# george-gca/sr-pytorch-lightning

Measured on AMD Instinct MI355X. Metric: SR training throughput, LR patches/s (48x48 LR x4, fwd+bwd+Adam), higher is better.
Workload: dtype bf16; 1 GPU; edsr_baseline x4, 48x48 LR patches, batch 256/GPU, train step (L1 + Adam); global_batch=256, parallelism=dp1, hip_graph=full

## Files before the change

### include/srk.h

```cpp
#ifndef SRK_H
#define SRK_H

#include <stdint.h>

#ifdef __cplusplus
extern "C" {
#endif

typedef void* srk_stream_t;

enum { SRK_BF16 = 0, SRK_F16 = 1, SRK_F32 = 2 };

enum {
  SRK_E_BADARG = -1,
  SRK_E_NODEV = -2
};

enum {
  SRK_OUT_NHWC = 0,
  SRK_OUT_NHWC_PS = 1,
  SRK_OUT_PLANAR = 2
};

typedef struct {
// ... 120 lines not shown
  int dtype;
} srk_pw_wgrad_args;
int srk_pw_wgrad_ranges(long long P, int Chid);
int srk_pw_wgrad(const srk_pw_wgrad_args* a, srk_stream_t stream);

typedef struct {
  const void* x; int x_pitch, x_coff; int x_ps;
  const void* dy; int dy_pitch, dy_coff; int dy_ps;
  int N, H, W;
  int Cin, Cout;
  int KH, KW;
  float* dwp;
  float* dbp;
  int nslabs;
  int dtype;
  int cout_real;
} srk_wgrad_args;
int srk_conv2d_wgrad(const srk_wgrad_args* a, srk_stream_t stream);
int srk_wgrad_slabs(const srk_wgrad_args* a);
int srk_wgrad_slab_cout(const srk_wgrad_args* a);

typedef struct {
  const float* dwp; const float* dbp;
  int nslabs;
  float* dw; float* db;
  int Cout, Cin, KH, KW;
  int CinP, CoutP;
  int ps_r;
  float scale;
  int accumulate;
} srk_wgrad_fin_args;
int srk_wgrad_finalize(const srk_wgrad_fin_args* a, srk_stream_t stream);

int srk_wgrad_group_ok(const srk_wgrad_args* a);
int srk_wgrad_group_job_bytes(void);
int srk_wgrad_group_plan(srk_wgrad_args* jobs, int n, float* scratch, void* table_host, int* block_job_host,
                         int* nblocks, long long* scratch_floats);
int srk_conv2d_wgrad_group(const void* table_dev, const int* block_job_dev, int nblocks, int dtype, srk_stream_t stream);
int srk_wgrad_finalize_group(const srk_wgrad_fin_args* table_dev, int n, int blocks_per_job, srk_stream_t stream);
int srk_upload_small(void* dst_dev, const void* src_host, long long nbytes, srk_stream_t stream);
int srk_upload_prepare(void);
int srk_upload_eager(void* dst_dev, const void* src_host, long long nbytes);
int srk_upload_fence(void);

typedef struct {
  const float* x;
  const float* sub;
  void* dst; int dst_pitch, dst_coff;
  int N, Cin, H, W, KH, KW;
  int Kstore;
  int dtype;
} srk_unfold_args;
int srk_unfold_nchw(const srk_unfold_args* a, srk_stream_t stream);

typedef struct {
  const float* src; void* dst; int dst_pitch, dst_coff;
  int N, C, H, W;
  int Cstore; int ps_r; float scale; int dtype;
} srk_to_nhwc_args;
int srk_nchw_to_nhwc(const srk_to_nhwc_args* a, srk_stream_t stream);

typedef struct {
  const void* src; int src_pitch, src_coff; float* dst;
  int N, C, H, W; int dtype;
} srk_to_nchw_args;
int srk_nhwc_to_nchw(const srk_to_nchw_args* a, srk_stream_t stream);

int srk_ca_splits(int N, int HW);
typedef struct {
  const void* t; int t_pitch, t_coff;
  const void* u; int u_pitch, u_coff;
  float* sums;
  int N, HW, C; int dtype;
} srk_ca_pool_args;
int srk_ca_pool(const srk_ca_pool_args* a, srk_stream_t stream);

typedef struct {
  const void* t; int t_pitch, t_coff;
  const void* res; int res_pitch, res_coff;
  const float* sums;
  const float* w1; const float* b1; const float* w2; const float* b2;
  float* s_out; float* z_out;
  void* out; int out_pitch, out_coff;
  int N, HW, C, Cr; int dtype;
  int sums_rows;
} srk_ca_apply_args;
int srk_ca_apply(const srk_ca_apply_args* a, srk_stream_t stream);

typedef struct {
  const void* g; int g_pitch, g_coff;
  const float* gsum;
  const float* sums; const float* s; const float* z;
  const float* w1; const float* w2;
  float* dw1; float* db1; float* dw2; float* db2;
  void* gt; int gt_pitch, gt_coff;
  int N, HW, C, Cr; int dtype;
  int sums_rows, gsum_rows;
} srk_ca_bwd_args;
int srk_ca_bwd_apply(const srk_ca_bwd_args* a, srk_stream_t stream);
typedef struct { const float* src; float* dst; int n; int k; } srk_rowsum_job;
int srk_rowsum_group(const srk_rowsum_job* table_dev, int njobs, int max_k, srk_stream_t stream);

typedef struct {
  const uint8_t* lr; const uint8_t* hr;
  int lr_h, lr_w, hr_h, hr_w;
  int top, left;
// ... 387 lines not shown
```

### sr-pytorch-lightning_amd/csrc/pack.hip

```cpp
#include <stdarg.h>
#include <string.h>
#include <mutex>
#include "srk_common.h"

static thread_local char g_err[512] = "";

void srk_set_error(const char* fmt, ...) {
  va_list ap;
  va_start(ap, fmt);
  vsnprintf(g_err, sizeof(g_err), fmt, ap);
  va_end(ap);
}

extern "C" const char* srk_last_error(void) { return g_err; }
thread_local const char* srk_kernel_name = "";
extern "C" const char* srk_last_kernel(void) { return srk_kernel_name; }
extern "C" int srk_version(void) { return 100; }
extern "C" int srk_device_cus(void) {
  int dev = 0;
  if (hipGetDevice(&dev) != hipSuccess) return 0;
  hipDeviceProp_t p;
  if (hipGetDeviceProperties(&p, dev) != hipSuccess) return 0;
  return p.multiProcessorCount;
}
// ... 371 lines not shown
  const int ncob = (a.CoutP + 63) / 64, ncib = (a.CinP + 1) / 2;
  for (int t = blockIdx.x; t < ncob * ncib; t += gridDim.x) {
    const int cob = t % ncob, cib = t / ncob;
    wgrad_finalize3x3_tile(a, tile, cib * 2, cob * 64);
  }
  if (a.db && a.dbp && blockIdx.x == 0) {
    const int ns = a.nslabs > 1 ? a.nslabs : 1;
    for (int cop = threadIdx.x; cop < a.Cout; cop += blockDim.x) {
      float u = 0.f;
#pragma unroll 8
      for (int sl = 0; sl < ns; ++sl) u += a.dbp[(size_t)sl * a.CoutP + cop];
      int co = cop;
      if (a.ps_r > 1) {
        const int r2p = a.ps_r * a.ps_r, Cc = a.Cout / r2p;
        const int ij = cop / Cc, c = cop - ij * Cc;
        co = c * r2p + ij;
      }
      const float v = a.scale * u;
      if (a.accumulate) a.db[co] += v; else a.db[co] = v;
    }
  }
}

template <int DT> __global__ void to_nhwc_kernel(const srk_to_nhwc_args a) {
  typedef DTraits<DT> Tr;
  typename Tr::elem* dst = reinterpret_cast<typename Tr::elem*>(a.dst);
  const int r = a.ps_r > 1 ? a.ps_r : 1, r2 = r * r;
  const int groups = a.Cstore / 4;
  const long long total = (long long)a.N * a.H * a.W * groups;
  const int Cs = a.C / r2;
  for (long long idx = (long long)blockIdx.x * blockDim.x + threadIdx.x; idx < total; idx += (long long)gridDim.x * blockDim.x) {
    const int g = (int)(idx % groups);
    long long p = idx / groups;
    const int x = (int)(p % a.W);
    p /= a.W;
    const int y = (int)(p % a.H);
    const int n = (int)(p / a.H);
    float v[4];
#pragma unroll
    for (int e = 0; e < 4; ++e) {
      const int c = g * 4 + e;
      float s = 0.f;
      if (c < a.C) {
        const int cs = c / r2, ij = c - cs * r2;
        const int si = ij / r, sj = ij - si * r;
        s = a.scale * a.src[((size_t)(n * Cs + cs) * (a.H * r) + y * r + si) * (a.W * r) + x * r + sj];
      }
      v[e] = s;
    }
    store4<DT>(dst + ((size_t)(n * a.H + y) * a.W + x) * a.dst_pitch + a.dst_coff + g * 4, v);
  }
}

template <int DT> __global__ void to_nhwc16_kernel(const srk_to_nhwc_args a) {
  typedef DTraits<DT> Tr;
  typename Tr::elem* dst = reinterpret_cast<typename Tr::elem*>(a.dst);
  const int r = a.ps_r > 1 ? a.ps_r : 1, r2 = r * r;
  const int Cs = a.C / r2;
  const long long total = (long long)a.N * a.H * a.W;
  for (long long p = (long long)blockIdx.x * blockDim.x + threadIdx.x; p < total; p += (long long)gridDim.x * blockDim.x) {
    const int x = (int)(p % a.W);
    long long q = p / a.W;
    const int y = (int)(q % a.H);
    const int n = (int)(q / a.H);
    float v[16];
#pragma unroll
    for (int c = 0; c < 16; ++c) {
      float s = 0.f;
      if (c < a.C) {
        const int cs = c / r2, ij = c - cs * r2;
        const int si = ij / r, sj = ij - si * r;
        s = a.scale * a.src[((size_t)(n * Cs + cs) * (a.H * r) + y * r + si) * (a.W * r) + x * r + sj];
      }
      v[c] = s;
    }
    typename Tr::elem* o = dst + (size_t)p * a.dst_pitch + a.dst_coff;
    if (Tr::IS16 && (a.dst_pitch & 7) == 0 && (a.dst_coff & 7) == 0) {
#pragma unroll
      for (int g = 0; g < 2; ++g) {
        i32x4 raw;
        raw.x = (int)pack2<DT>(v[8 * g + 0], v[8 * g + 1]); raw.y = (int)pack2<DT>(v[8 * g + 2], v[8 * g + 3]);
        raw.z = (int)pack2<DT>(v[8 * g + 4], v[8 * g + 5]); raw.w = (int)pack2<DT>(v[8 * g + 6], v[8 * g + 7]);
        *reinterpret_cast<i32x4*>(o + 8 * g) = raw;
      }
    } else {
#pragma unroll
      for (int g = 0; g < 4; ++g) store4<DT>(o + 4 * g, v + 4 * g);
    }
  }
}

template <int DT> __global__ void to_nchw_kernel(const srk_to_nchw_args a) {
  typedef DTraits<DT> Tr;
  const typename Tr::elem* src = reinterpret_cast<const typename Tr::elem*>(a.src);
  const long long total = (long long)a.N * a.C * a.H * a.W;
  for (long long idx = (long long)blockIdx.x * blockDim.x + threadIdx.x; idx < total; idx += (long long)gridDim.x * blockDim.x) {
    const int x = (int)(idx % a.W);
    long long t = idx / a.W;
    const int y = (int)(t % a.H);
    t /= a.H;
    const int c = (int)(t % a.C);
    const int n = (int)(t / a.C);
    a.dst[idx] = Tr::to_f32(src[((size_t)(n * a.H + y) * a.W + x) * a.src_pitch + a.src_coff + c]);
  }
}

template <int DT> __global__ void unfold_kernel(const srk_unfold_args a) {
  typedef DTraits<DT> Tr;
  typename Tr::elem* dst = reinterpret_cast<typename Tr::elem*>(a.dst);
  const int groups = a.Kstore / 4, taps = a.KH * a.KW, K = a.Cin * taps;
  const int ph = a.KH / 2, pw = a.KW / 2;
  const long long total = (long long)a.N * a.H * a.W * groups;
  for (long long idx = (long long)blockIdx.x * blockDim.x + threadIdx.x; idx < total; idx += (long long)gridDim.x * blockDim.x) {
    const int g = (int)(idx % groups);
    long long p = idx / groups;
    const int x = (int)(p % a.W);
    p /= a.W;
    const int y = (int)(p % a.H);
    const int n = (int)(p / a.H);
    float v[4];
#pragma unroll
    for (int e = 0; e < 4; ++e) {
      const int k = g * 4 + e;
      float s = 0.f;
      if (k < K) {
        const int ci = k / taps, t = k - ci * taps;
        const int kh = t / a.KW, kw = t - kh * a.KW;
        const int yy = y + kh - ph, xx = x + kw - pw;
        if (yy >= 0 && yy < a.H && xx >= 0 && xx < a.W) {
          s = a.x[((size_t)(n * a.Cin + ci) * a.H + yy) * a.W + xx];
          if (a.sub) s -= a.sub[ci];
        }
      }
      v[e] = s;
    }
    store4<DT>(dst + ((size_t)(n * a.H + y) * a.W + x) * a.dst_pitch + a.dst_coff + g * 4, v);
  }
}

inline int grid_for(long long total, int block) {
// ... 91 lines not shown
constexpr int kMaxDev = 64;
std::mutex g_upload_mu;
hipStream_t g_upload_stream[kMaxDev] = {};
int upload_stream_of_current_device(hipStream_t* out, bool create) {
  int dev = -1;
  hipError_t e = hipGetDevice(&dev);
  if (e != hipSuccess || dev < 0 || dev >= kMaxDev) { srk_set_error("srk_upload: hipGetDevice: %s (device %d)", hipGetErrorString(e), dev); return e != hipSuccess ? (int)e : SRK_E_BADARG; }
  std::lock_guard<std::mutex> lock(g_upload_mu);
  if (!g_upload_stream[dev] && create) {
    e = hipStreamCreateWithFlags(&g_upload_stream[dev], hipStreamNonBlocking);
    if (e != hipSuccess) { g_upload_stream[dev] = nullptr; srk_set_error("srk_upload_prepare: %s", hipGetErrorString(e)); return (int)e; }
  }
  *out = g_upload_stream[dev];
  return 0;
}
}
extern "C" int srk_upload_prepare(void) {
  hipStream_t st = nullptr;
  return upload_stream_of_current_device(&st, true);
}
extern "C" int srk_upload_eager(void* dst_dev, const void* src_host, long long nbytes) {
  hipStream_t st = nullptr;
  const int rc = upload_stream_of_current_device(&st, false);
  if (rc != 0) return rc;
  SRK_CHECK_ARG(st != nullptr, "srk_upload_eager: call srk_upload_prepare() on this device first (outside the capture)");
  return srk_upload_small(dst_dev, src_host, nbytes, reinterpret_cast<srk_stream_t>(st));
}
extern "C" int srk_upload_fence(void) {
  hipStream_t st = nullptr;
  const int rc = upload_stream_of_current_device(&st, false);
  if (rc != 0) return rc;
  if (!st) return 0;
  const hipError_t e = hipStreamSynchronize(st);
  if (e != hipSuccess) { srk_set_error("srk_upload_fence: %s", hipGetErrorString(e)); return (int)e; }
  return 0;
}

extern "C" int srk_wgrad_finalize_group(const srk_wgrad_fin_args* table_dev, int n, int blocks_per_job, srk_stream_t stream) {
  SRK_CHECK_ARG(table_dev && n > 0 && n <= 65535, "srk_wgrad_finalize_group: bad table (%d entries)", n);
  const int bx = blocks_per_job < 1 ? 1 : (blocks_per_job > 2048 ? 2048 : blocks_per_job);
  hipLaunchKernelGGL(wgrad_finalize_group_kernel, dim3(bx, n), dim3(256), 0, reinterpret_cast<hipStream_t>(stream), table_dev);
  SRK_LAUNCH_CHECK();
  return 0;
}

extern "C" int srk_nchw_to_nhwc(const srk_to_nhwc_args* a, srk_stream_t stream) {
  SRK_CHECK_ARG(a && a->src && a->dst, "srk_nchw_to_nhwc: null pointer");
  const int r = a->ps_r > 1 ? a->ps_r : 1;
  SRK_CHECK_ARG(a->Cstore % 4 == 0 && a->Cstore >= a->C && a->C % (r * r) == 0 && a->dst_pitch % 4 == 0 && a->dst_coff % 4 == 0,
                "srk_nchw_to_nhwc: C=%d Cstore=%d r=%d", a->C, a->Cstore, r);
  hipStream_t st = reinterpret_cast<hipStream_t>(stream);
  if (a->Cstore == 16) {
    const long long px = (long long)a->N * a->H * a->W;
    const int g16 = (int)((px + 255) / 256 > 8192 ? 8192 : (px + 255) / 256);
    switch (a->dtype) {
      case SRK_BF16: hipLaunchKernelGGL(to_nhwc16_kernel<SRK_BF16>, dim3(g16), dim3(256), 0, st, *a); break;
      case SRK_F16: hipLaunchKernelGGL(to_nhwc16_kernel<SRK_F16>, dim3(g16), dim3(256), 0, st, *a); break;
      case SRK_F32: hipLaunchKernelGGL(to_nhwc16_kernel<SRK_F32>, dim3(g16), dim3(256), 0, st, *a); break;
      default: SRK_CHECK_ARG(false, "srk_nchw_to_nhwc: dtype %d", a->dtype);
    }
    SRK_LAUNCH_CHECK();
    return 0;
  }
  const long long total = (long long)a->N * a->H * a->W * (a->Cstore / 4);
  const int grid = grid_for(total, 256);
  switch (a->dtype) {
    case SRK_BF16: hipLaunchKernelGGL(to_nhwc_kernel<SRK_BF16>, dim3(grid), dim3(256), 0, st, *a); break;
    case SRK_F16: hipLaunchKernelGGL(to_nhwc_kernel<SRK_F16>, dim3(grid), dim3(256), 0, st, *a); break;
    case SRK_F32: hipLaunchKernelGGL(to_nhwc_kernel<SRK_F32>, dim3(grid), dim3(256), 0, st, *a); break;
    default: SRK_CHECK_ARG(false, "srk_nchw_to_nhwc: dtype %d", a->dtype);
  }
  SRK_LAUNCH_CHECK();
  return 0;
}

extern "C" int srk_nhwc_to_nchw(const srk_to_nchw_args* a, srk_stream_t stream) {
  SRK_CHECK_ARG(a && a->src && a->dst, "srk_nhwc_to_nchw: null pointer");
  const long long total = (long long)a->N * a->C * a->H * a->W;
  hipStream_t st = reinterpret_cast<hipStream_t>(stream);
  const int grid = grid_for(total, 256);
  switch (a->dtype) {
    case SRK_BF16: hipLaunchKernelGGL(to_nchw_kernel<SRK_BF16>, dim3(grid), dim3(256), 0, st, *a); break;
    case SRK_F16: hipLaunchKernelGGL(to_nchw_kernel<SRK_F16>, dim3(grid), dim3(256), 0, st, *a); break;
    case SRK_F32: hipLaunchKernelGGL(to_nchw_kernel<SRK_F32>, dim3(grid), dim3(256), 0, st, *a); break;
    default: SRK_CHECK_ARG(false, "srk_nhwc_to_nchw: dtype %d", a->dtype);
  }
  SRK_LAUNCH_CHECK();
  return 0;
}

template <int DT> __global__ __launch_bounds__(256) void unfold3x3c3_kernel(const srk_unfold_args a) {
  typedef DTraits<DT> Tr;
  static_assert(Tr::IS16, "16-bit storage");
  typename Tr::elem* dst = reinterpret_cast<typename Tr::elem*>(a.dst);
  const long long total = (long long)a.N * a.H * a.W;
  const float sub[3] = {a.sub ? a.sub[0] : 0.f, a.sub ? a.sub[1] : 0.f, a.sub ? a.sub[2] : 0.f};
  for (long long p = (long long)blockIdx.x * 256 + threadIdx.x; p < total; p += (long long)gridDim.x * 256) {
    const int x = (int)(p % a.W);
    const long long q = p / a.W;
    const int y = (int)(q % a.H);
    const int n = (int)(q / a.H);
    float v[32];
#pragma unroll
    for (int ci = 0; ci < 3; ++ci) {
      const float* const plane = a.x + (size_t)(n * 3 + ci) * a.H * a.W;
#pragma unroll
// ... 52 lines not shown
```

### sr-pytorch-lightning_amd/ops.py

```python
import weakref

import torch

from . import _lib as L
from .packing import *
from .packing import _DT, _TLS, _f32c, _group_for, _knob, _need_gpu, _ptr, _roundup, _stream, _tok


def _pitch(t):
    n, h, w, c = t.shape
    p = t.stride(2) if w > 1 else (t.stride(1) if h > 1 else (t.stride(0) if n > 1 else c))
    if w > 1 and h > 1:
        assert t.stride(1) == w * p, "NHWC view must be dense in W"
    if h > 1 and n > 1:
        assert t.stride(0) == h * w * p, "NHWC view must be dense in H"
    assert c == 1 or t.stride(3) == 1, "channels must be innermost"
    return p


_ADDR_LIMIT = 0x7fff0000


def _batch_chunks(n, *tensors):
    worst = 0
# ... 221 lines not shown
            assert c % 16 == 0, "fused PixelShuffle store needs C % 16 == 0"
            out = torch.empty((n, h * ps_r, wd * ps_r, c), dtype=x.dtype, device=x.device)
            conv_raw(x, pk, N=n, H=h, W=wd, Cin=cinp, Cout=cout, out=out, out_mode=L.OUT_NHWC_PS, ps_r=ps_r,
                     scale=scale, res=res)
        else:
            out = torch.empty((n, h, wd, pad16(cout)), dtype=x.dtype, device=x.device)
            conv_raw(x, pk, N=n, H=h, W=wd, Cin=cinp, Cout=out.shape[3], out=out, scale=scale, res=res)
        ctx.save_for_backward(x, w)
        ctx.cfg = (scale, ps_r, b is not None, res is not None)
        ctx.wb = (w, b)
        ctx.pg = _tok()
        ctx.gacc = x.__dict__.get("_srk_gacc")
        return out

    @staticmethod
    def backward(ctx, g):
        x, w = ctx.saved_tensors
        scale, ps_r, has_b, has_res = ctx.cfg
        g = g.contiguous()
        n, h, wd, cinp = x.shape
        cout, cin, k, _ = w.shape
        coutp = pad16(cout)
        gx = gw = gb = None
        if ctx.needs_input_grad[0]:
            pkd = pack_conv(w, None, x.dtype, dgrad=True, ps_r=ps_r, token=ctx.pg)
            if ctx.gacc is not None and ps_r <= 1:
                gx, add = ctx.gacc[0].grad_dest(ctx.gacc[1])
                conv_raw(g, pkd, N=n, H=h, W=wd, Cin=coutp, Cout=cinp, out=gx, scale=scale, use_bias=False, res=gx if add else None)
            else:
                gx = torch.empty_like(x)
                parked = None
                if ctx.link is not None and ctx.link.g is not None:
                    parked, ctx.link.g = ctx.link.g, None
                conv_raw(g, pkd, N=n, H=h, W=wd, Cin=coutp, Cout=cinp, out=gx, scale=scale, x_ps=ps_r, use_bias=False, res=parked)
        if ctx.needs_input_grad[1] or ctx.needs_input_grad[2]:
            gw, gb = wgrad(x, g, wparam=ctx.wb[0], bparam=ctx.wb[1], N=n, H=h, W=wd, Cin=cinp, Cout=coutp, k=k,
                           w_shape=tuple(w.shape), ps_r=ps_r, scale=scale, dy_ps=ps_r, want_bias=has_b)
            gw = gw if ctx.needs_input_grad[1] else None
        return gx, gw, gb, (g if has_res else None), None, None, None


def conv(x, w, b, *, res=None, scale=1.0, ps_r=0, link=None):
    return ConvFn.apply(x, w, b, res, float(scale), int(ps_r), link)


class HeadConvFn(torch.autograd.Function):

    @staticmethod
    def forward(ctx, x, w, b, sub, dtype):
        _need_gpu(x)
        cout, cin, k, _ = w.shape
        n, c, h, wd = x.shape
        assert c == cin
        xu = unfold_raw(x, sub, k, dtype)
        pk = _pack_head(w, b, dtype)
        out = torch.empty((n, h, wd, pad16(cout)), dtype=dtype, device=x.device)
        conv_raw(xu, pk, N=n, H=h, W=wd, Cin=xu.shape[3], Cout=out.shape[3], out=out)
        ctx.save_for_backward(xu, w)
        ctx.has_b = b is not None
        return out

    @staticmethod
    def backward(ctx, g):
        xu, w = ctx.saved_tensors
        g = g.contiguous()
        n, h, wd, kp = xu.shape
        gw = gb = None
        if ctx.needs_input_grad[1] or ctx.needs_input_grad[2]:
            gw, gb = wgrad_raw(xu, g, N=n, H=h, W=wd, Cin=kp, Cout=g.shape[3], k=1, w_shape=tuple(w.shape),
                               want_bias=ctx.has_b)
            gw = gw if ctx.needs_input_grad[1] else None
        return None, gw, gb, None, None


def _pack_head(w, b, dtype):
    return pack_conv(w, b, dtype, as_1x1=True)


def head_conv(x, w, b, sub, dtype):
    return HeadConvFn.apply(x, w, b, sub, dtype)


class TailConvFn(torch.autograd.Function):

    @staticmethod
    def forward(ctx, x, w, b, res, post_add, ps_r):
        _need_gpu(x)
        n, h, wd, cinp = x.shape
        cout, cin, k, _ = w.shape
        r = ps_r if ps_r > 1 else 1
        pk = pack_conv(w, b, x.dtype)
        out = torch.empty((n, cout // (r * r), h * r, wd * r), dtype=torch.float32, device=x.device)
        resc = None if res is None else _f32c(res)
        conv_raw(x, pk, N=n, H=h, W=wd, Cin=cinp, Cout=cout, out=out, out_mode=L.OUT_PLANAR, ps_r=ps_r,
                 res=resc, post_add=post_add)
        ctx.save_for_backward(x, w)
        ctx.cfg = (ps_r, b is not None, res is not None)
        ctx.wb = (w, b)
        ctx.pg = _tok()
        return out

    @staticmethod
    def backward(ctx, g):
        x, w = ctx.saved_tensors
        ps_r, has_b, has_res = ctx.cfg
        n, h, wd, cinp = x.shape
        cout, cin, k, _ = w.shape
        dy = to_nhwc(g, x.dtype, ps_r=ps_r)
        gx = gw = gb = None
        if ctx.needs_input_grad[0]:
            pkd = pack_conv(w, None, x.dtype, dgrad=True, token=ctx.pg)
            gx = torch.empty_like(x)
            conv_raw(dy, pkd, N=n, H=h, W=wd, Cin=dy.shape[3], Cout=cinp, out=gx, use_bias=False)
        if ctx.needs_input_grad[1] or ctx.needs_input_grad[2]:
            gw, gb = wgrad(x, dy, wparam=ctx.wb[0], bparam=ctx.wb[1], N=n, H=h, W=wd, Cin=cinp, Cout=dy.shape[3], k=k,
                           w_shape=tuple(w.shape), want_bias=has_b)
            gw = gw if ctx.needs_input_grad[1] else None
        return gx, gw, gb, (g if has_res else None), None, None


def tail_conv(x, w, b, *, res=None, post_add=None, ps_r=0):
    return TailConvFn.apply(x, w, b, res, post_add, int(ps_r))


class SkipConvFn(torch.autograd.Function):

    @staticmethod
    def forward(ctx, x, w, b, sub, ps_r, dtype):
        _need_gpu(x)
# ... 930 lines not shown
```

### sr-pytorch-lightning_amd/csrc/conv_wgrad.hip

```cpp
#include <stdlib.h>
#include <mutex>
#include "srk_common.h"

namespace {

template <int DT, int KS> struct WgCfg {
  typedef DTraits<DT> Tr;
  static constexpr int CH = Tr::CH;
  static constexpr int ESZ = 16 / CH;
  static constexpr int CBLK = 128 / ESZ;
  static constexpr int RB = CBLK / 32;
  static constexpr int PAIRS = RB * RB;
  static constexpr int KGROUPS = 4 / PAIRS;
  static constexpr int NT = 256;
  static constexpr int NTAPS = KS * KS;
  static constexpr int PAD = KS / 2;
  static constexpr int TIN = 16 + KS - 1;
  static constexpr int PITCH = (TIN + 1) & ~1;
  static constexpr int XS_BYTES = TIN * PITCH * 128;
  static constexpr int DYS_BYTES = 256 * 128;
  static constexpr int LDS_BYTES = XS_BYTES + DYS_BYTES;
  static constexpr int XPIECES = TIN * TIN * 8;
  static constexpr int DYPIECES = 256 * 8;
};
// ... 308 lines not shown
      for (int t = 0; t < 9; ++t) {
        const int kh = t / KS, kw = t - kh * KS;
        acc[t] = Tr::mma(xf[(y + kh) & 3][kw], bf, acc[t]);
        if (t == 1 && 2 * y < NPK && more) dma_x_piece(nxt, 2 * y);
        if (t == 4 && 2 * y + 1 < NPK && more) dma_x_piece(nxt, 2 * y + 1);
        if (t == 7 && y < NDK && more) dma_d_piece(nxt, y);
      }
      bf = bfn;
      __builtin_amdgcn_sched_barrier(0);
    }
  }

  {
    const int co = cob * 64 + cbk * 32 + (lane & 31);
    const int hq = lane >> 5;
    const size_t slab_elems = (size_t)9 * a.Cin * a.Cout;
    const __amdgpu_buffer_rsrc_t srs =
        __builtin_amdgcn_make_buffer_rsrc(a.dwp + (size_t)slot * slab_elems, 0, (unsigned)(slab_elems * 4), 0x00020000);
    const int ci0 = cib * 64 + rb * 32 + 4 * hq;
#pragma unroll
    for (int t = 0; t < 9; ++t) {
#pragma unroll
      for (int e = 0; e < 16; ++e) {
        const int ci = ci0 + (e & 3) + 8 * (e >> 2);
        const unsigned voff = (ci < a.Cin && co < a.Cout) ? (unsigned)(((t * a.Cin + ci) * a.Cout + co) * 4) : 0x80000000u;
        __builtin_amdgcn_raw_buffer_store_b32(__float_as_uint(acc[t][e]), srs, voff, 0, 0);
      }
    }
  }
  if (do_bias) {
    float* const bred = reinterpret_cast<float*>(smem);
    __syncthreads();
#pragma unroll
    for (int e = 0; e < 8; ++e) bred[tid * 8 + e] = bsum8[e];
    __syncthreads();
    if (tid < 64) {
      const int ch = tid >> 3, e = tid & 7;
      float t = 0.f;
      for (int p0 = 0; p0 < 32; ++p0) t += bred[((p0 << 3) + (ch ^ swz(p0 & 15))) * 8 + e];
      const int c = cob * 64 + tid;
      if (c < a.Cout) a.dbp[(size_t)slot * a.Cout + c] = t;
    }
  }
}


constexpr int WS_TH = 8;

SRK_DEV void add_f32_unpacked(float& s, float v) { asm("v_add_f32_e32 %0, %0, %1" : "+v"(s) : "v"(v)); }

#ifndef SRK_WG_STAMPS
#define SRK_WG_STAMPS 0
#endif
#ifndef SRK_WG_HELPER_SLEEP
#define SRK_WG_HELPER_SLEEP 0
#endif
#ifndef SRK_WG_COMPUTE_PRIO
#define SRK_WG_COMPUTE_PRIO 0
#endif
constexpr int WS8_THREADS = 512;

template <int DT, bool BIAS>
SRK_DEV void wgrad_ws_body8(const srk_wgrad_args& a, const int slot, const int cib, const int cob, const int tilesX, const int tilesY,
                           const unsigned x_bytes, const unsigned dy_bytes, const int tq, const int trem, char* const smem, const bool single) {
  typedef WgCfg<DT, 3> C;
  typedef typename C::Tr Tr;
  constexpr int CH = C::CH, KS = 3, GT = 256, ESZ = C::ESZ;
  constexpr int TH = WS_TH, NBUF = 4, AHEAD = NBUF - 1;
  constexpr int XPIECES = (TH + 2) * C::TIN * 8;
  constexpr int NPK = (XPIECES + GT - 1) / GT;
  constexpr int NDK = TH * 16 * 8 / GT;
  constexpr int PPT = NPK + NDK;
  constexpr int XS_PAD = NPK * GT * 16, DYS = TH * 16 * 128;
  constexpr int BUF_BYTES = XS_PAD + DYS;
  static_assert(NBUF * BUF_BYTES <= 160 * 1024, "the ring must fit the LDS");

  const int wave = __builtin_amdgcn_readfirstlane((int)threadIdx.x >> 6);
  const int t0 = slot * tq + min(slot, trem);
  const int nt = tq + (slot < trem ? 1 : 0);
#if SRK_WG_STAMPS
  unsigned long long* const stamp = (single && slot == 0 && cib == 0 && cob == 0 && (threadIdx.x & 255) == 0 && a.dbp)
                                        ? reinterpret_cast<unsigned long long*>(a.dbp + (size_t)a.nslabs * a.Cout) + (wave >> 2) * 64 : nullptr;
#define SRK_GSTAMP(i) do { if (stamp && it < 32) stamp[it * 2 + (i)] = __builtin_amdgcn_s_memtime(); } while (0)
#else
#define SRK_GSTAMP(i) do { } while (0)
#endif

  if (wave >= 4) {
    const int tid = (int)threadIdx.x - GT, hw = wave - 4;
    const int H = a.H, W = a.W;
    const int nch_x = a.Cin / CH, nch_d = a.Cout / CH;
    const i32x4 xrs = make_rsrc4(a.x, x_bytes), drs = make_rsrc4(a.dy, dy_bytes);
    const unsigned lds0 = lds_addr_of(smem);
    int pconst[NPK], pyx[NPK];
#pragma unroll
    for (int k = 0; k < NPK; ++k) {
      const int i = tid + k * GT;
      const int sl = i & 7, p = i >> 3;
      const int iy = p / C::TIN, ix = p - iy * C::TIN;
      const int c = cib * 8 + (sl ^ swz(ix));
      pconst[k] = (((iy - 1) * W + (ix - 1)) * a.x_pitch + a.x_coff + c * CH) * ESZ;
      pyx[k] = (i < XPIECES && c < nch_x) ? (((iy - 1) & 0xffff) | ((ix - 1) << 16)) : (int)0x7fff7fff;
    }
    const int rd = a.dy_ps > 1 ? a.dy_ps : 1;
    const int d_ix = (tid >> 3) & 15, d_iy0 = tid >> 7;
    const int d_c = cob * 8 + ((tid & 7) ^ swz(d_ix));
    const bool d_cok = d_c < nch_d;
    int dconst, dkstride;
    {
      const int Csd = a.Cout / (rd * rd);
      const int k0 = d_c * CH;
      const int ij = k0 / Csd, c0 = k0 - ij * Csd;
      const int si = ij / rd, sj = ij - si * rd;
      dconst = (((d_iy0 * rd + si) * (W * rd) + d_ix * rd + sj) * a.dy_pitch + a.dy_coff + c0) * ESZ;
      dkstride = 2 * rd * (W * rd) * a.dy_pitch * ESZ;
    }
    struct TileAddr { int y0, x0, xbase, dbase; bool colok, live; unsigned Xb; };
    int nx_tX = t0 % tilesX, nx_tY = (t0 / tilesX) % tilesY, nx_n = (t0 / tilesX) / tilesY;
    auto dma_tile = [&](int it_) {
      TileAddr t;
      t.live = it_ < nt;
      t.y0 = nx_tY * TH; t.x0 = nx_tX * 16;
      const int row = nx_n * H + t.y0;
      t.xbase = ((row * W + t.x0) * a.x_pitch) * ESZ;
      t.dbase = ((row * rd * (W * rd) + t.x0 * rd) * a.dy_pitch) * ESZ;
      t.colok = t.live && d_cok && (t.x0 + d_ix < W);
      t.Xb = lds0 + (unsigned)((it_ & (NBUF - 1)) * BUF_BYTES);
      const bool wx = nx_tX + 1 == tilesX;
      nx_tX = wx ? 0 : nx_tX + 1;
      nx_tY += wx ? 1 : 0;
      const bool wy = nx_tY == tilesY;
      nx_tY = wy ? 0 : nx_tY;
      nx_n += wy ? 1 : 0;
#pragma unroll
      for (int k = 0; k < NPK; ++k) {
        const int gy = t.y0 + (int)(short)(pyx[k] & 0xffff), gx = t.x0 + (pyx[k] >> 16);
        const bool ok = t.live && (unsigned)gy < (unsigned)H && (unsigned)gx < (unsigned)W;
        const unsigned voff = ok ? (unsigned)(t.xbase + pconst[k]) : 0x80000000u;
        dma16_hidden(xrs, voff, __builtin_amdgcn_readfirstlane(t.Xb + ((k * GT + hw * 64) << 4)));
        if (SRK_WG_HELPER_SLEEP) __builtin_amdgcn_s_sleep(SRK_WG_HELPER_SLEEP);
      }
#pragma unroll
      for (int k = 0; k < NDK; ++k) {
        const bool ok = t.colok && (t.y0 + d_iy0 + 2 * k < H);
        const unsigned voff = ok ? (unsigned)(t.dbase + dconst + k * dkstride) : 0x80000000u;
        dma16_hidden(drs, voff, __builtin_amdgcn_readfirstlane(t.Xb + XS_PAD + ((k * GT + hw * 64) << 4)));
        if (SRK_WG_HELPER_SLEEP) __builtin_amdgcn_s_sleep(SRK_WG_HELPER_SLEEP);
      }
    };
    float bsum8[8] = {0.f, 0.f, 0.f, 0.f, 0.f, 0.f, 0.f, 0.f};

#pragma unroll
    for (int k = 0; k < AHEAD; ++k) dma_tile(k);
    asm volatile("s_waitcnt vmcnt(%0)" :: "n"((AHEAD - 1) * PPT) : "memory");
    __builtin_amdgcn_s_barrier();
#pragma unroll 1
    for (int it = 0; it < nt; ++it) {
      SRK_GSTAMP(0);
      dma_tile(it + AHEAD);
      if (BIAS) {
        const char* const Ds = smem + (it & (NBUF - 1)) * BUF_BYTES + XS_PAD;
#pragma unroll
        for (int k = 0; k < NDK; ++k) {
          const i32x4 braw = lds_read16(Ds + ((tid + 256 * k) << 4));
#pragma unroll
          for (int i = 0; i < 4; ++i) {
            const uint32_t w = (uint32_t)braw[i];
            add_f32_unpacked(bsum8[2 * i], Tr::to_f32((uint16_t)(w & 0xffff)));
            add_f32_unpacked(bsum8[2 * i + 1], Tr::to_f32((uint16_t)(w >> 16)));
          }
        }
      }
      asm volatile("s_waitcnt lgkmcnt(0)\n\ts_waitcnt vmcnt(%0)" :: "n"((AHEAD - 1) * PPT) : "memory");
      SRK_GSTAMP(1);
      __builtin_amdgcn_s_barrier();
    }
    asm volatile("s_waitcnt vmcnt(0)" ::: "memory");
    if (BIAS) {
      float* const bred = reinterpret_cast<float*>(smem);
      __syncthreads();
#pragma unroll
      for (int e = 0; e < 8; ++e) bred[tid * 8 + e] = bsum8[e];
      __syncthreads();
      if (tid < 64) {
        const int ch = tid >> 3, e = tid & 7;
        float t = 0.f;
        for (int p0 = 0; p0 < 32; ++p0) t += bred[((p0 << 3) + (ch ^ swz(p0 & 15))) * 8 + e];
        const int c = cob * 64 + tid;
        if (c < a.Cout) a.dbp[(size_t)slot * a.Cout + c] = t;
      }
    }
    return;
  }

  const int tid = threadIdx.x, lane = tid & 63;
  const int rb = wave >> 1, cbk = wave & 1;
  f32x16 acc[9];
#pragma unroll
  for (int t = 0; t < 9; ++t)
#pragma unroll
    for (int e = 0; e < 16; ++e) acc[t][e] = 0.f;
  int xoff[KS][2], doff[2];
#pragma unroll
  for (int kw = 0; kw < KS; ++kw) {
    xoff[kw][0] = tr_lane_off(kw, 0, rb, lane);
    xoff[kw][1] = tr_lane_off(kw, 1, rb, lane);
  }
  doff[0] = tr_lane_off(0, 0, cbk, lane);
  doff[1] = tr_lane_off(0, 1, cbk, lane);
  i32x4 pxf[3][KS], pbf;
  auto read_first_frags = [&](const char* Xb) {
    const char* const Db = Xb + XS_PAD;
    pbf = tr_read2(Db + doff[0], Db + doff[1]);
#pragma unroll
    for (int rr = 0; rr < 3; ++rr)
#pragma unroll
      for (int kw = 0; kw < KS; ++kw)
        pxf[rr][kw] = tr_read2(Xb + xoff[kw][0] + rr * (C::PITCH * 128), Xb + xoff[kw][1] + rr * (C::PITCH * 128));
  };

  if (SRK_WG_COMPUTE_PRIO) __builtin_amdgcn_s_setprio(SRK_WG_COMPUTE_PRIO);
  asm volatile("" ::: "memory");
  __builtin_amdgcn_s_barrier();
  asm volatile("" ::: "memory");
  read_first_frags(smem);
#pragma unroll 1
  for (int it = 0; it < nt; ++it) {
    SRK_GSTAMP(0);
    const char* const Xs = smem + (it & (NBUF - 1)) * BUF_BYTES;
    const char* const Ds = Xs + XS_PAD;
    const char* const Xn = smem + ((it + 1) & (NBUF - 1)) * BUF_BYTES;
    i32x4 xf[4][KS];
#pragma unroll
    for (int rr = 0; rr < 3; ++rr)
#pragma unroll
      for (int kw = 0; kw < KS; ++kw) xf[rr][kw] = pxf[rr][kw];
    i32x4 bf = pbf;
#pragma unroll
    for (int y = 0; y < TH; ++y) {
      i32x4 bfn = bf;
      if (y + 1 < TH) {
        const int nr = y + 3;
#pragma unroll
        for (int kw = 0; kw < KS; ++kw)
          xf[nr & 3][kw] = tr_read2(Xs + xoff[kw][0] + nr * (C::PITCH * 128), Xs + xoff[kw][1] + nr * (C::PITCH * 128));
        bfn = tr_read2(Ds + doff[0] + (y + 1) * (16 * 128), Ds + doff[1] + (y + 1) * (16 * 128));
      }
#pragma unroll
      for (int t = 0; t < 9; ++t) {
        const int kh = t / KS, kw = t - kh * KS;
        acc[t] = Tr::mma(xf[(y + kh) & 3][kw], bf, acc[t]);
        if (y == TH - 1 && t == 0) {
          __builtin_amdgcn_sched_barrier(0);
          asm volatile("s_waitcnt lgkmcnt(0)" ::: "memory");
          SRK_GSTAMP(1);
          __builtin_amdgcn_s_barrier();
          __builtin_amdgcn_sched_barrier(0);
        }
        if (y == TH - 1 && t == 1) {
          __builtin_amdgcn_sched_barrier(0);
          read_first_frags(Xn);
        }
      }
      bf = bfn;
      __builtin_amdgcn_sched_barrier(0);
    }
  }

  {
    const int co = cob * 64 + cbk * 32 + (lane & 31);
    const int hq = lane >> 5;
    const size_t slab_elems = (size_t)9 * a.Cin * a.Cout;
    const __amdgpu_buffer_rsrc_t srs =
        __builtin_amdgcn_make_buffer_rsrc(a.dwp + (size_t)slot * slab_elems, 0, (unsigned)(slab_elems * 4), 0x00020000);
    const int ci0 = cib * 64 + rb * 32 + 4 * hq;
#pragma unroll
    for (int t = 0; t < 9; ++t) {
#pragma unroll
      for (int e = 0; e < 16; ++e) {
        const int ci = ci0 + (e & 3) + 8 * (e >> 2);
        const unsigned voff = (ci < a.Cin && co < a.Cout) ? (unsigned)(((t * a.Cin + ci) * a.Cout + co) * 4) : 0x80000000u;
        __builtin_amdgcn_raw_buffer_store_b32(__float_as_uint(acc[t][e]), srs, voff, 0, 0);
      }
    }
  }
  if (BIAS) {
    __syncthreads();
    __syncthreads();
  }
#undef SRK_GSTAMP
}

template <int DT>
SRK_DEV void wgrad_ws_run8(const srk_wgrad_args& a, const int slot, const int cib, const int cob, const int tilesX, const int tilesY,
                          const unsigned x_bytes, const unsigned dy_bytes, const int tq, const int trem, char* const smem, const bool single) {
  if (a.dbp != nullptr && cib == 0) wgrad_ws_body8<DT, true>(a, slot, cib, cob, tilesX, tilesY, x_bytes, dy_bytes, tq, trem, smem, single);
  else wgrad_ws_body8<DT, false>(a, slot, cib, cob, tilesX, tilesY, x_bytes, dy_bytes, tq, trem, smem, single);
}

template <int DT>
__global__ __launch_bounds__(256, 1) void conv_wgrad_ws_kernel(const srk_wgrad_args a, int tilesX, int tilesY,
                                                                unsigned x_bytes, unsigned dy_bytes, int tq, int trem) {
  extern __shared__ __attribute__((aligned(16))) char smem[];
  wgrad_ws_body16<DT>(a, blockIdx.x, blockIdx.y, blockIdx.z, tilesX, tilesY, x_bytes, dy_bytes, tq, trem, smem);
}
template <int DT>
__global__ __launch_bounds__(WS8_THREADS, 2) void conv_wgrad_ws8_kernel(const srk_wgrad_args a, int tilesX, int tilesY,
                                                                         unsigned x_bytes, unsigned dy_bytes, int tq, int trem) {
  extern __shared__ __attribute__((aligned(16))) char smem[];
  wgrad_ws_run8<DT>(a, blockIdx.x, blockIdx.y, blockIdx.z, tilesX, tilesY, x_bytes, dy_bytes, tq, trem, smem, true);
}

struct WgJob {
  srk_wgrad_args a;
  int tilesX, tilesY;
  unsigned x_bytes, dy_bytes;
  int tq, trem;
  int ncib, ncob;
// ... 583 lines not shown
```

Before: 49670 LR patches/s.

## Fuse head conv unfold with MFMA conv and add vectorized r=2 NHWC repack

Result: no change. 50120 LR patches/s, median of 6 (+0.9%).

```diff
diff --git a/include/srk.h b/include/srk.h
--- a/include/srk.h
+++ b/include/srk.h
@@ -196,6 +196,18 @@
   int dtype;
 } srk_unfold_args;
 int srk_unfold_nchw(const srk_unfold_args* a, srk_stream_t stream);
+
+typedef struct {
+  const float* x;
+  const float* sub;
+  const void* wpk;
+  const float* bias;
+  void* out;
+  void* xu;
+  int N, H, W;
+  int dtype;
+} srk_head_conv_args;
+int srk_head_conv3x3(const srk_head_conv_args* a, srk_stream_t stream);
 
 typedef struct {
   const float* src; void* dst; int dst_pitch, dst_coff;
diff --git a/sr-pytorch-lightning_amd/csrc/head_conv.hip b/sr-pytorch-lightning_amd/csrc/head_conv.hip
--- /dev/null
+++ b/sr-pytorch-lightning_amd/csrc/head_conv.hip
@@ -0,0 +1,171 @@
+#include "srk_common.h"
+
+namespace {
+
+typedef __attribute__((ext_vector_type(4))) unsigned int u32x4;
+
+constexpr int HC_T = 16;
+constexpr int HC_TIN = HC_T + 2;
+constexpr int HC_STAGE = 3 * HC_TIN * HC_TIN;
+constexpr int HC_NT = 256;
+constexpr int HC_SV = (HC_STAGE + HC_NT - 1) / HC_NT;
+constexpr int HC_WG_PER_CU = 3;
+
+SRK_DEV int col_slot(int p, int c) { return c ^ ((p >> 2) & 3); }
+
+template <int DT>
+__global__ __launch_bounds__(HC_NT, HC_WG_PER_CU) void head_conv3x3_kernel(const srk_head_conv_args a, int tilesX, int tilesY, int ntiles) {
+  typedef DTraits<DT> Tr;
+  typedef typename Tr::elem elem;
+  static_assert(Tr::IS16, "16-bit storage");
+  __shared__ float S[HC_STAGE];
+  __shared__ __attribute__((aligned(16))) char Cl[HC_NT * 64];
+  __shared__ __attribute__((aligned(16))) float Bs[64];
+
+  const int tid = threadIdx.x;
+  const int lane = tid & 63;
+  const int wave = __builtin_amdgcn_readfirstlane(tid >> 6);
+  const int r = lane & 31, h = lane >> 5;
+  const int H = a.H, W = a.W;
+  const float sub[3] = {a.sub ? a.sub[0] : 0.f, a.sub ? a.sub[1] : 0.f, a.sub ? a.sub[2] : 0.f};
+
+  i32x4 af[2][2];
+  const elem* const wg = reinterpret_cast<const elem*>(a.wpk);
+#pragma unroll
+  for (int ks = 0; ks < 2; ++ks)
+#pragma unroll
+    for (int cb = 0; cb < 2; ++cb) af[ks][cb] = gload16(wg + (size_t)(((2 * ks + h) * 64 + cb * 32 + r) * 8));
+  if (tid < 64) Bs[tid] = a.bias ? a.bias[tid] : 0.f;
+
+  auto fetch = [&](int t, float (&sv)[HC_SV]) {
+    const int tX = t % tilesX;
+    const int q = t / tilesX;
+    const int tY = q % tilesY, n = q / tilesY;
+#pragma unroll
+    for (int u = 0; u < HC_SV; ++u) {
+      const int i = tid + u * HC_NT;
+      float v = 0.f;
+      if (i < HC_STAGE) {
+        const int ci = i / (HC_TIN * HC_TIN), rem = i - ci * (HC_TIN * HC_TIN);
+        const int iy = rem / HC_TIN, ix = rem - iy * HC_TIN;
+        const int gy = tY * HC_T + iy - 1, gx = tX * HC_T + ix - 1;
+        if (gy >= 0 && gy < H && gx >= 0 && gx < W) v = a.x[((size_t)(n * 3 + ci) * H + gy) * W + gx] - sub[ci];
+      }
+      sv[u] = v;
+    }
+  };
+
+  const int ty = tid >> 4, tx = tid & 15;
+  const int px = r & 15, qi = px & 3;
+
+  float sv[HC_SV];
+  int t = blockIdx.x;
+  if (t < ntiles) fetch(t, sv);
+  for (; t < ntiles; t += gridDim.x) {
+    const int tX = t % tilesX;
+    const int q = t / tilesX;
+    const int tY = q % tilesY, n = q / tilesY;
+    const int y0 = tY * HC_T, x0 = tX * HC_T;
+
+#pragma unroll
+    for (int u = 0; u < HC_SV; ++u)
+      if (tid + u * HC_NT < HC_STAGE) S[tid + u * HC_NT] = sv[u];
+    __syncthreads();
+    if (t + (int)gridDim.x < ntiles) fetch(t + gridDim.x, sv);
+
+    {
+      float v[32];
+#pragma unroll
+      for (int ci = 0; ci < 3; ++ci)
+#pragma unroll
+        for (int kh = 0; kh < 3; ++kh)
+#pragma unroll
+          for (int kw = 0; kw < 3; ++kw) v[ci * 9 + kh * 3 + kw] = S[(ci * HC_TIN + ty + kh) * HC_TIN + tx + kw];
+#pragma unroll
+      for (int k = 27; k < 32; ++k) v[k] = 0.f;
+#pragma unroll
+      for (int c = 0; c < 4; ++c) {
+        i32x4 raw;
+        raw.x = (int)pack2<DT>(v[8 * c + 0], v[8 * c + 1]); raw.y = (int)pack2<DT>(v[8 * c + 2], v[8 * c + 3]);
+        raw.z = (int)pack2<DT>(v[8 * c + 4], v[8 * c + 5]); raw.w = (int)pack2<DT>(v[8 * c + 6], v[8 * c + 7]);
+        lds_write16(Cl + tid * 64 + (col_slot(tid, c) << 4), raw);
+      }
+    }
+    __syncthreads();
+
+    if (a.xu) {
+      elem* const xu = reinterpret_cast<elem*>(a.xu);
+#pragma unroll
+      for (int u = 0; u < 4; ++u) {
+        const int i = tid + u * HC_NT;
+        const int p = i >> 2, c = i & 3;
+        const int gy = y0 + (p >> 4), gx = x0 + (p & 15);
+        if (gy < H && gx < W)
+          *reinterpret_cast<i32x4*>(xu + ((size_t)(n * H + gy) * W + gx) * 32 + c * 8) = lds_read16(Cl + p * 64 + (col_slot(p, c) << 4));
+      }
+    }
+
+    elem* const out = reinterpret_cast<elem*>(a.out);
+    const int gxb = x0 + (px & ~3);
+#pragma unroll
+    for (int pb = 0; pb < 2; ++pb) {
+      f32x16 acc[2];
+#pragma unroll
+      for (int cb = 0; cb < 2; ++cb)
+#pragma unroll
+        for (int i = 0; i < 4; ++i) {
+          const f32x4 b = *reinterpret_cast<const f32x4*>(Bs + 4 * h + cb * 32 + 8 * i);
+          acc[cb][4 * i + 0] = b.x; acc[cb][4 * i + 1] = b.y; acc[cb][4 * i + 2] = b.z; acc[cb][4 * i + 3] = b.w;
+        }
+      const int p = (wave * 2 + pb) * 32 + r;
+      i32x4 bf[2];
+#pragma unroll
+      for (int ks = 0; ks < 2; ++ks) bf[ks] = lds_read16(Cl + p * 64 + (col_slot(p, 2 * ks + h) << 4));
+#pragma unroll
+      for (int ks = 0; ks < 2; ++ks)
+#pragma unroll
+        for (int cb = 0; cb < 2; ++cb) acc[cb] = Tr::mma(af[ks][cb], bf[ks], acc[cb]);
+
+      const int gy = y0 + (wave * 2 + pb) * 2 + (r >> 4);
+      uint32_t P[4][4];
+#pragma unroll
+      for (int k = 0; k < 4; ++k)
+#pragma unroll
+        for (int d = 0; d < 4; ++d) P[k][d] = pack2<DT>(acc[k >> 1][8 * (k & 1) + 2 * d], acc[k >> 1][8 * (k & 1) + 2 * d + 1]);
+      quad_transpose8_dpp(P[0][0], P[1][0], P[2][0], P[3][0], P[0][1], P[1][1], P[2][1], P[3][1]);
+      quad_transpose8_dpp(P[0][2], P[1][2], P[2][2], P[3][2], P[0][3], P[1][3], P[2][3], P[3][3]);
+      if (gy < H) {
+        elem* const o = out + ((size_t)(n * H + gy) * W + gxb) * 64 + 32 * h + 8 * qi;
+#pragma unroll
+        for (int j = 0; j < 4; ++j)
+          if (gxb + j < W) *reinterpret_cast<u32x4*>(o + (size_t)j * 64) = u32x4{P[j][0], P[j][1], P[j][2], P[j][3]};
+      }
+    }
+  }
+}
+
+}
+
+extern "C" int srk_head_conv3x3(const srk_head_conv_args* a, srk_stream_t stream) {
+  SRK_CHECK_ARG(a && a->x && a->wpk && a->out, "srk_head_conv3x3: null pointer");
+  SRK_CHECK_ARG(a->N > 0 && a->H > 0 && a->W > 0, "srk_head_conv3x3: bad dims N=%d H=%d W=%d", a->N, a->H, a->W);
+  SRK_CHECK_ARG(a->dtype == SRK_BF16 || a->dtype == SRK_F16, "srk_head_conv3x3: dtype %d (16-bit storage only)", a->dtype);
+  SRK_CHECK_ARG(((reinterpret_cast<uintptr_t>(a->wpk) | reinterpret_cast<uintptr_t>(a->out) | reinterpret_cast<uintptr_t>(a->xu) |
+                  reinterpret_cast<uintptr_t>(a->bias)) & 15) == 0,
+                "srk_head_conv3x3: wpk, bias, out and xu must be 16-byte aligned");
+  SRK_CHECK_ARG((long long)a->N * a->H * a->W < 0x7fffffffLL, "srk_head_conv3x3: %lld pixels", (long long)a->N * a->H * a->W);
+  const int tilesX = (a->W + HC_T - 1) / HC_T, tilesY = (a->H + HC_T - 1) / HC_T;
+  const long long ntiles = (long long)a->N * tilesX * tilesY;
+  SRK_CHECK_ARG(ntiles < 0x40000000LL, "srk_head_conv3x3: %lld tiles", ntiles);
+  static const int cus = [] { int c = srk_device_cus(); return c > 0 ? c : 256; }();
+  const long long cap = (long long)cus * HC_WG_PER_CU;
+  long long passes = (ntiles + cap - 1) / cap;
+  if (passes < 2 && ntiles >= 2) passes = 2;
+  const unsigned grid = (unsigned)((ntiles + passes - 1) / passes);
+  hipStream_t st = reinterpret_cast<hipStream_t>(stream);
+  srk_kernel_name = "head_conv3x3";
+  if (a->dtype == SRK_BF16) hipLaunchKernelGGL(head_conv3x3_kernel<SRK_BF16>, dim3(grid), dim3(HC_NT), 0, st, *a, tilesX, tilesY, (int)ntiles);
+  else hipLaunchKernelGGL(head_conv3x3_kernel<SRK_F16>, dim3(grid), dim3(HC_NT), 0, st, *a, tilesX, tilesY, (int)ntiles);
+  SRK_LAUNCH_CHECK();
+  return 0;
+}
diff --git a/sr-pytorch-lightning_amd/csrc/pack.hip b/sr-pytorch-lightning_amd/csrc/pack.hip
--- a/sr-pytorch-lightning_amd/csrc/pack.hip
+++ b/sr-pytorch-lightning_amd/csrc/pack.hip
@@ -447,6 +447,22 @@
   }
 }
 
+template <int DT> SRK_DEV void store_px16(const srk_to_nhwc_args& a, typename DTraits<DT>::elem* o, const float (&v)[16]) {
+  typedef DTraits<DT> Tr;
+  if (Tr::IS16 && (a.dst_pitch & 7) == 0 && (a.dst_coff & 7) == 0) {
+#pragma unroll
+    for (int g = 0; g < 2; ++g) {
+      i32x4 raw;
+      raw.x = (int)pack2<DT>(v[8 * g + 0], v[8 * g + 1]); raw.y = (int)pack2<DT>(v[8 * g + 2], v[8 * g + 3]);
+      raw.z = (int)pack2<DT>(v[8 * g + 4], v[8 * g + 5]); raw.w = (int)pack2<DT>(v[8 * g + 6], v[8 * g + 7]);
+      *reinterpret_cast<i32x4*>(o + 8 * g) = raw;
+    }
+  } else {
+#pragma unroll
+    for (int g = 0; g < 4; ++g) store4<DT>(o + 4 * g, v + 4 * g);
+  }
+}
+
 template <int DT> __global__ void to_nhwc16_kernel(const srk_to_nhwc_args a) {
   typedef DTraits<DT> Tr;
   typename Tr::elem* dst = reinterpret_cast<typename Tr::elem*>(a.dst);
@@ -469,18 +485,43 @@
       }
       v[c] = s;
     }
-    typename Tr::elem* o = dst + (size_t)p * a.dst_pitch + a.dst_coff;
-    if (Tr::IS16 && (a.dst_pitch & 7) == 0 && (a.dst_coff & 7) == 0) {
-#pragma unroll
-      for (int g = 0; g < 2; ++g) {
-        i32x4 raw;
-        raw.x = (int)pack2<DT>(v[8 * g + 0], v[8 * g + 1]); raw.y = (int)pack2<DT>(v[8 * g + 2], v[8 * g + 3]);
-        raw.z = (int)pack2<DT>(v[8 * g + 4], v[8 * g + 5]); raw.w = (int)pack2<DT>(v[8 * g + 6], v[8 * g + 7]);
-        *reinterpret_cast<i32x4*>(o + 8 * g) = raw;
-      }
-    } else {
-#pragma unroll
-      for (int g = 0; g < 4; ++g) store4<DT>(o + 4 * g, v + 4 * g);
+    store_px16<DT>(a, dst + (size_t)p * a.dst_pitch + a.dst_coff, v);
+  }
+}
+
+template <int DT> __global__ __launch_bounds__(256) void to_nhwc16_r2_kernel(const srk_to_nhwc_args a) {
+  typedef DTraits<DT> Tr;
+  typename Tr::elem* dst = reinterpret_cast<typename Tr::elem*>(a.dst);
+  const int Cs = a.C / 4;
+  const size_t Ws = (size_t)a.W * 2, plane = (size_t)a.H * 2 * Ws;
+  const long long total = (long long)a.N * a.H * a.W, stride = (long long)gridDim.x * 256;
+  for (long long p0 = (long long)blockIdx.x * 256 + threadIdx.x; p0 < total; p0 += 2 * stride) {
+    f32x2 q[2][8];
+#pragma unroll
+    for (int u = 0; u < 2; ++u) {
+      const long long p = p0 + u * stride;
+      const bool ok = p < total;
+      const int x = (int)(p % a.W);
+      const long long t = p / a.W;
+      const int y = (int)(t % a.H);
+      const int n = (int)(t / a.H);
+      const float* const s = a.src + (size_t)n * Cs * plane + (size_t)(2 * y) * Ws + 2 * x;
+#pragma unroll
+      for (int cs = 0; cs < 4; ++cs)
+#pragma unroll
+        for (int si = 0; si < 2; ++si)
+          q[u][cs * 2 + si] = (ok && cs < Cs) ? *reinterpret_cast<const f32x2*>(s + cs * plane + si * Ws) : f32x2{0.f, 0.f};
+    }
+#pragma unroll
+    for (int u = 0; u < 2; ++u) {
+      const long long p = p0 + u * stride;
+      if (p >= total) break;
+      float v[16];
+#pragma unroll
+      for (int cs = 0; cs < 4; ++cs)
+#pragma unroll
+        for (int e = 0; e < 4; ++e) v[cs * 4 + e] = cs < Cs ? a.scale * q[u][cs * 2 + (e >> 1)][e & 1] : 0.f;
+      store_px16<DT>(a, dst + (size_t)p * a.dst_pitch + a.dst_coff, v);
     }
   }
 }
@@ -678,6 +719,17 @@
   hipStream_t st = reinterpret_cast<hipStream_t>(stream);
   if (a->Cstore == 16) {
     const long long px = (long long)a->N * a->H * a->W;
+    if (a->ps_r == 2 && (reinterpret_cast<uintptr_t>(a->src) & 7) == 0) {
+      const int g2 = (int)((px + 511) / 512 > 8192 ? 8192 : (px + 511) / 512);
+      switch (a->dtype) {
+        case SRK_BF16: hipLaunchKernelGGL(to_nhwc16_r2_kernel<SRK_BF16>, dim3(g2), dim3(256), 0, st, *a); break;
+        case SRK_F16: hipLaunchKernelGGL(to_nhwc16_r2_kernel<SRK_F16>, dim3(g2), dim3(256), 0, st, *a); break;
+        case SRK_F32: hipLaunchKernelGGL(to_nhwc16_r2_kernel<SRK_F32>, dim3(g2), dim3(256), 0, st, *a); break;
+        default: SRK_CHECK_ARG(false, "srk_nchw_to_nhwc: dtype %d", a->dtype);
+      }
+      SRK_LAUNCH_CHECK();
+      return 0;
+    }
     const int g16 = (int)((px + 255) / 256 > 8192 ? 8192 : (px + 255) / 256);
     switch (a->dtype) {
       case SRK_BF16: hipLaunchKernelGGL(to_nhwc16_kernel<SRK_BF16>, dim3(g16), dim3(256), 0, st, *a); break;
diff --git a/sr-pytorch-lightning_amd/ops.py b/sr-pytorch-lightning_amd/ops.py
--- a/sr-pytorch-lightning_amd/ops.py
+++ b/sr-pytorch-lightning_amd/ops.py
@@ -297,10 +297,16 @@
         cout, cin, k, _ = w.shape
         n, c, h, wd = x.shape
         assert c == cin
-        xu = unfold_raw(x, sub, k, dtype)
         pk = _pack_head(w, b, dtype)
         out = torch.empty((n, h, wd, pad16(cout)), dtype=dtype, device=x.device)
-        conv_raw(xu, pk, N=n, H=h, W=wd, Cin=xu.shape[3], Cout=out.shape[3], out=out)
+        if _head_fused_ok(x, w, pk, out):
+            xu = None
+            if ctx.needs_input_grad[1] or ctx.needs_input_grad[2]:
+                xu = torch.empty((n, h, wd, pk.KinP), dtype=dtype, device=x.device)
+            head_conv_raw(x, sub, pk, out, xu)
+        else:
+            xu = unfold_raw(x, sub, k, dtype)
+            conv_raw(xu, pk, N=n, H=h, W=wd, Cin=xu.shape[3], Cout=out.shape[3], out=out)
         ctx.save_for_backward(xu, w)
         ctx.has_b = b is not None
         return out
@@ -320,6 +326,27 @@
 
 def _pack_head(w, b, dtype):
     return pack_conv(w, b, dtype, as_1x1=True)
+
+
+_HEAD_FUSED_OFF = _knob("SRK_NO_HEAD_FUSED", "0") == "1"
+
+
+def _head_fused_ok(x, w, pk, out):
+    if _HEAD_FUSED_OFF or out.dtype not in (torch.bfloat16, torch.float16) or tuple(w.shape[1:]) != (3, 3, 3):
+        return False
+    if out.shape[3] != 64 or pk.CoutP != 64 or pk.KinP != 32 or out.numel() == 0 or out.numel() // 64 >= 2 ** 30:
+        return False
+    return not isinstance(L.load().srk_head_conv3x3, L._Absent)
+
+
+def head_conv_raw(x, sub, pk, out, xu=None):
+    _need_gpu(x)
+    n, _, h, wd = x.shape
+    xs = _f32c(x)
+    a = L.HeadConvArgs(x=xs.data_ptr(), sub=_ptr(sub), wpk=pk.wpk.data_ptr(), bias=_ptr(pk.bias), out=out.data_ptr(), xu=_ptr(xu),
+                       N=n, H=h, W=wd, dtype=_DT[out.dtype])
+    L.call("srk_head_conv3x3", a, _stream())
+    return out
 
 
 def head_conv(x, w, b, sub, dtype):
```

## Interleave wgrad LDS transpose reads with MFMAs using a 5-slot register ring

Applied to the files above, without the earlier changes.

After: 49630 LR patches/s before, 50020 LR patches/s after, median of 6. No clear change (+0.8%).

```diff
diff --git a/sr-pytorch-lightning_amd/csrc/conv_wgrad.hip b/sr-pytorch-lightning_amd/csrc/conv_wgrad.hip
--- a/sr-pytorch-lightning_amd/csrc/conv_wgrad.hip
+++ b/sr-pytorch-lightning_amd/csrc/conv_wgrad.hip
@@ -384,12 +384,6 @@
 #ifndef SRK_WG_STAMPS
 #define SRK_WG_STAMPS 0
 #endif
-#ifndef SRK_WG_HELPER_SLEEP
-#define SRK_WG_HELPER_SLEEP 0
-#endif
-#ifndef SRK_WG_COMPUTE_PRIO
-#define SRK_WG_COMPUTE_PRIO 0
-#endif
 constexpr int WS8_THREADS = 512;
 
 template <int DT, bool BIAS>
@@ -470,14 +464,12 @@
         const bool ok = t.live && (unsigned)gy < (unsigned)H && (unsigned)gx < (unsigned)W;
         const unsigned voff = ok ? (unsigned)(t.xbase + pconst[k]) : 0x80000000u;
         dma16_hidden(xrs, voff, __builtin_amdgcn_readfirstlane(t.Xb + ((k * GT + hw * 64) << 4)));
-        if (SRK_WG_HELPER_SLEEP) __builtin_amdgcn_s_sleep(SRK_WG_HELPER_SLEEP);
       }
 #pragma unroll
       for (int k = 0; k < NDK; ++k) {
         const bool ok = t.colok && (t.y0 + d_iy0 + 2 * k < H);
         const unsigned voff = ok ? (unsigned)(t.dbase + dconst + k * dkstride) : 0x80000000u;
         dma16_hidden(drs, voff, __builtin_amdgcn_readfirstlane(t.Xb + XS_PAD + ((k * GT + hw * 64) << 4)));
-        if (SRK_WG_HELPER_SLEEP) __builtin_amdgcn_s_sleep(SRK_WG_HELPER_SLEEP);
       }
     };
     float bsum8[8] = {0.f, 0.f, 0.f, 0.f, 0.f, 0.f, 0.f, 0.f};
@@ -532,70 +524,92 @@
   for (int t = 0; t < 9; ++t)
 #pragma unroll
     for (int e = 0; e < 16; ++e) acc[t][e] = 0.f;
-  int xoff[KS][2], doff[2];
-#pragma unroll
-  for (int kw = 0; kw < KS; ++kw) {
-    xoff[kw][0] = tr_lane_off(kw, 0, rb, lane);
-    xoff[kw][1] = tr_lane_off(kw, 1, rb, lane);
-  }
-  doff[0] = tr_lane_off(0, 0, cbk, lane);
-  doff[1] = tr_lane_off(0, 1, cbk, lane);
-  i32x4 pxf[3][KS], pbf;
-  auto read_first_frags = [&](const char* Xb) {
-    const char* const Db = Xb + XS_PAD;
-    pbf = tr_read2(Db + doff[0], Db + doff[1]);
-#pragma unroll
-    for (int rr = 0; rr < 3; ++rr)
-#pragma unroll
-      for (int kw = 0; kw < KS; ++kw)
-        pxf[rr][kw] = tr_read2(Xb + xoff[kw][0] + rr * (C::PITCH * 128), Xb + xoff[kw][1] + rr * (C::PITCH * 128));
+  constexpr int NSLOT = 5, XROW = C::PITCH * 128, DROW = 16 * 128;
+  static_assert((TH + 2) % NSLOT == 0 && TH % 2 == 0, "the slot phase must repeat every tile");
+  static_assert(XS_PAD + TH * DROW + 2 * 128 < 65536, "row offsets must fit the DS immediate");
+  const unsigned lds0 = lds_addr_of(smem);
+  unsigned xa[KS][2], da[2];
+#pragma unroll
+  for (int kw = 0; kw < KS; ++kw)
+#pragma unroll
+    for (int rd = 0; rd < 2; ++rd) xa[kw][rd] = lds0 + (unsigned)tr_lane_off(kw, rd, rb, lane);
+#pragma unroll
+  for (int rd = 0; rd < 2; ++rd) da[rd] = lds0 + (unsigned)(XS_PAD + tr_lane_off(0, rd, cbk, lane));
+  auto pin_addrs = [&]() {
+#pragma unroll
+    for (int kw = 0; kw < KS; ++kw)
+#pragma unroll
+      for (int rd = 0; rd < 2; ++rd) asm volatile("" : "+v"(xa[kw][rd]));
+#pragma unroll
+    for (int rd = 0; rd < 2; ++rd) asm volatile("" : "+v"(da[rd]));
   };
-
-  if (SRK_WG_COMPUTE_PRIO) __builtin_amdgcn_s_setprio(SRK_WG_COMPUTE_PRIO);
+  pin_addrs();
+  auto lds_tr2 = [](unsigned a0, unsigned a1) {
+    typedef __attribute__((address_space(3))) i16x4 lds_i16x4;
+    const i16x4 lo = __builtin_amdgcn_ds_read_tr16_b64_v4i16((lds_i16x4*)(size_t)a0);
+    const i16x4 hi = __builtin_amdgcn_ds_read_tr16_b64_v4i16((lds_i16x4*)(size_t)a1);
+    const i32x2 l2 = __builtin_bit_cast(i32x2, lo), h2 = __builtin_bit_cast(i32x2, hi);
+    return i32x4{l2.x, l2.y, h2.x, h2.y};
+  };
+  i32x4 xf[NSLOT][KS], bf[2];
+  auto read_x = [&](int r, int kw) { xf[r % NSLOT][kw] = lds_tr2(xa[kw][0] + r * XROW, xa[kw][1] + r * XROW); };
+  auto read_d = [&](int y) { bf[y & 1] = lds_tr2(da[0] + y * DROW, da[1] + y * DROW); };
+
   asm volatile("" ::: "memory");
   __builtin_amdgcn_s_barrier();
   asm volatile("" ::: "memory");
-  read_first_frags(smem);
+  read_d(0);
+  __builtin_amdgcn_sched_barrier(0);
+#pragma unroll
+  for (int r = 0; r < 3; ++r)
+#pragma unroll
+    for (int kw = 0; kw < KS; ++kw)
+      if (r < 2 || kw == 0) {
+        read_x(r, kw);
+        __builtin_amdgcn_sched_barrier(0);
+      }
+  auto step_addrs = [&](int to_next) {
+#pragma unroll
+    for (int k = 0; k < KS; ++k)
+#pragma unroll
+      for (int rd = 0; rd < 2; ++rd) xa[k][rd] += (unsigned)to_next;
+#pragma unroll
+    for (int rd = 0; rd < 2; ++rd) da[rd] += (unsigned)to_next;
+    pin_addrs();
+  };
 #pragma unroll 1
   for (int it = 0; it < nt; ++it) {
     SRK_GSTAMP(0);
-    const char* const Xs = smem + (it & (NBUF - 1)) * BUF_BYTES;
-    const char* const Ds = Xs + XS_PAD;
-    const char* const Xn = smem + ((it + 1) & (NBUF - 1)) * BUF_BYTES;
-    i32x4 xf[4][KS];
-#pragma unroll
-    for (int rr = 0; rr < 3; ++rr)
-#pragma unroll
-      for (int kw = 0; kw < KS; ++kw) xf[rr][kw] = pxf[rr][kw];
-    i32x4 bf = pbf;
+    const int to_next = ((it + 1) & (NBUF - 1)) ? BUF_BYTES : -(NBUF - 1) * BUF_BYTES;
 #pragma unroll
     for (int y = 0; y < TH; ++y) {
-      i32x4 bfn = bf;
-      if (y + 1 < TH) {
-        const int nr = y + 3;
-#pragma unroll
-        for (int kw = 0; kw < KS; ++kw)
-          xf[nr & 3][kw] = tr_read2(Xs + xoff[kw][0] + nr * (C::PITCH * 128), Xs + xoff[kw][1] + nr * (C::PITCH * 128));
-        bfn = tr_read2(Ds + doff[0] + (y + 1) * (16 * 128), Ds + doff[1] + (y + 1) * (16 * 128));
-      }
 #pragma unroll
       for (int t = 0; t < 9; ++t) {
         const int kh = t / KS, kw = t - kh * KS;
-        acc[t] = Tr::mma(xf[(y + kh) & 3][kw], bf, acc[t]);
-        if (y == TH - 1 && t == 0) {
+        acc[t] = Tr::mma(xf[(y + kh) % NSLOT][kw], bf[y & 1], acc[t]);
+        if (y == 0) {
+          if (t < 2) read_x(2, t + 1);
+          else if (t == 2) read_d(1);
+          else if (t & 1) read_x(3, t / 2 - 1);
+        } else if (y < TH - 2) {
+          if (t == 0) read_d(y + 1);
+          else if ((t & 1) == 0 && t <= 6) read_x(y + 3, t / 2 - 1);
+        } else if (y == TH - 2) {
+          if (t < 3) read_x(y + 3, t);
+          else if (t == 3) read_d(y + 1);
+        } else if (t == 0) {
           __builtin_amdgcn_sched_barrier(0);
           asm volatile("s_waitcnt lgkmcnt(0)" ::: "memory");
           SRK_GSTAMP(1);
           __builtin_amdgcn_s_barrier();
           __builtin_amdgcn_sched_barrier(0);
-        }
-        if (y == TH - 1 && t == 1) {
-          __builtin_amdgcn_sched_barrier(0);
-          read_first_frags(Xn);
-        }
-      }
-      bf = bfn;
-      __builtin_amdgcn_sched_barrier(0);
+          step_addrs(to_next);
+        } else if (t == 1) read_d(0);
+        else if (t <= 4) read_x(0, t - 2);
+        else if (t <= 7) read_x(1, t - 5);
+        else read_x(2, 0);
+        __builtin_amdgcn_sched_barrier(0);
+      }
     }
   }
 
```
